# lhaippp/DMHomo

Measured on AMD Instinct MI355X. Metric: sampled images/sec (128x128, s_step=32), higher is better.
Workload: dtype f32; 1 GPU; DGM CFG-Unet dim=64 128x128 bs=25/GPU s_step=32 cond_scale=3 (BASELINE configs[1]); global_batch=25, cfg_mode=streams, hip_graph=True, weights=seeded random init

## Files before the change

dmhomo_amd/csrc/linattn_fused.hip:

```cpp

#include "common.h"

typedef _Float16 half8 __attribute__((ext_vector_type(8)));
typedef _Float16 half4 __attribute__((ext_vector_type(4)));
typedef float float4v __attribute__((ext_vector_type(4)));

#define LA_PART (32 + 32 + 1024)

#ifdef DMH_STAMPS
__device__ int g_la_ablate = 0;
extern "C" int dmh_la_set_ablate(int v) {
  return hipMemcpyToSymbol(HIP_SYMBOL(g_la_ablate), &v, sizeof(int)) == hipSuccess ? 0 : -1;
}
#define LA_ABL_LOAD() const int la_abl = g_la_ablate
#define LA_ABL(bit) ((la_abl >> (bit)) & 1)
#else
#define LA_ABL_LOAD() constexpr int la_abl = 0
#define LA_ABL(bit) 0
#endif

namespace {
constexpr int KC = 32;

__device__ __forceinline__ void la_split2(float x0, float x1, float s, unsigned& h, unsigned& r, int cheap) {
  if (cheap) {
    float t0 = x0 * s, t1 = x1 * s;
    asm("v_cvt_pk_f16_f32 %0, %1, %2" : "=v"(h) : "v"(t0), "v"(t1));
    r = 0u;
  } else {
    dmh_split2(x0, x1, s, h, r);
  }
}
__device__ __forceinline__ void la_split8(const float (&x)[8], float s, dmh_half8& h, dmh_half8& r, int cheap) {
  if (cheap) {
    uint4 hh, rr = make_uint4(0u, 0u, 0u, 0u);
    la_split2(x[0], x[1], s, hh.x, rr.x, 1);
    la_split2(x[2], x[3], s, hh.y, rr.y, 1);
    la_split2(x[4], x[5], s, hh.z, rr.z, 1);
    la_split2(x[6], x[7], s, hh.w, rr.w, 1);
    asm volatile("s_nop 3" : "+v"(hh.x), "+v"(hh.y), "+v"(hh.z), "+v"(hh.w));
    h = __builtin_bit_cast(dmh_half8, hh);
    r = __builtin_bit_cast(dmh_half8, rr);
  } else {
    dmh_split8(x, s, h, r);
  }
}
constexpr int PITCH = 160;
constexpr int TP = 64;
constexpr int TILE_BYTES = TP * PITCH;

__device__ __forceinline__ unsigned absbits(float x) { return __float_as_uint(x) & 0x7fffffffu; }

template <int NBUF>
struct Stager {
  const float* xb;
  const float* g;
  int C, n, p0;
  int c4, pix0;
  float mean[2], rstd[2];
  bool ok[2];
  float4 v[2];
  float4 gq;
  float sc, inv_sc;
  int seq = 0;
  int abl = 0;

  __device__ __forceinline__ void init_scale() {
    float m = 0.f;
    for (int i = threadIdx.x & 63; i < C; i += 64) m = fmaxf(m, fabsf(g[i]));
#pragma unroll
    for (int off = 32; off; off >>= 1) m = fmaxf(m, __shfl_xor(m, off));
    const float bound = m * sqrtf((float)C);
    const int e = min(max((int)(__builtin_amdgcn_readfirstlane(__float_as_uint(bound)) >> 23) & 0xff, 16), 254);
    sc = __uint_as_float((unsigned)(268 - e) << 23);
    inv_sc = __uint_as_float((unsigned)(e - 14) << 23);
  }
  __device__ __forceinline__ void begin_tile(const float* stats_b, int p0_) {
    p0 = p0_;
#pragma unroll
    for (int i = 0; i < 2; ++i) {
      const int pix = p0 + pix0 + 32 * i;
      ok[i] = pix < n;
      const int pc = (abl & 8) ? pix0 : (ok[i] ? pix : n - 1);
      mean[i] = stats_b[(size_t)pc * 2 + 0];
      rstd[i] = stats_b[(size_t)pc * 2 + 1];
    }
  }
  __device__ __forceinline__ void issue(int ch) {
#pragma unroll
    for (int i = 0; i < 2; ++i) {
      const int pix = p0 + pix0 + 32 * i;
      const int pc = (abl & 8) ? pix0 : (pix < n ? pix : n - 1);
      v[i] = ld4(xb + (size_t)pc * C + ch * KC + c4 * 4);
    }
    gq = ld4(g + ch * KC + c4 * 4);
  }
  __device__ __forceinline__ unsigned char* stage(unsigned char* tiles) {
    unsigned char* tile = tiles + (NBUF == 2 ? (seq & 1) * TILE_BYTES : 0);
    ++seq;
    if (NBUF == 1) __syncthreads();
#pragma unroll
    for (int i = 0; i < 2; ++i) {
      float4 x = v[i];
      if (ok[i]) {
        x.x = (x.x - mean[i]) * rstd[i] * gq.x;
        x.y = (x.y - mean[i]) * rstd[i] * gq.y;
        x.z = (x.z - mean[i]) * rstd[i] * gq.z;
        x.w = (x.w - mean[i]) * rstd[i] * gq.w;
      } else {
        x = make_float4(0.f, 0.f, 0.f, 0.f);
      }
      uint2 h1, h2;
      la_split2(x.x, x.y, sc, h1.x, h2.x, abl & 1);
      la_split2(x.z, x.w, sc, h1.y, h2.y, abl & 1);
      unsigned char* dst = tile + (pix0 + 32 * i) * PITCH + c4 * 8;
      *reinterpret_cast<uint2*>(dst) = h1;
      *reinterpret_cast<uint2*>(dst + 64) = h2;
    }
    __syncthreads();
    return tile;
  }
  __device__ __forceinline__ float inv_scale() const { return inv_sc; }
};

__device__ __forceinline__ void dmh_raw_barrier() {
  asm volatile("" ::: "memory");
  __builtin_amdgcn_s_barrier();
  asm volatile("" ::: "memory");
}

struct RingStager {
  static constexpr int RD = 2;
  static constexpr int UNIT = TP * 64 * 4;
  static constexpr int STATS_SLOTS = 4;
  static constexpr int BYTES = RD * UNIT + STATS_SLOTS * TP * 8;
  const float* xb;
  const float* stats_b;
  int n, p0w, U;
  int c4, pix0, lane, wave;
  unsigned char* ring;
  unsigned ring_lds;
  float4 gq[2];
  float sc, inv_sc;
  int seq = 0;
  int abl = 0;

  __device__ __forceinline__ void init(const float* x_b, const float* stats_b_, const float* g, int n_, int p0w_, int tiles,
                                       unsigned char* ring_) {
    xb = x_b;
    stats_b = stats_b_;
    n = n_;
    p0w = p0w_;
    const int left = (n - p0w + TP - 1) / TP;
    U = left < tiles ? left : tiles;
    lane = threadIdx.x & 63;
    wave = __builtin_amdgcn_readfirstlane(threadIdx.x >> 6);
    c4 = threadIdx.x & 7;
    pix0 = threadIdx.x >> 3;
    ring = ring_;
    ring_lds = (unsigned)(size_t)ring_;
    float m = fabsf(g[lane]);
#pragma unroll
    for (int off = 32; off; off >>= 1) m = fmaxf(m, __shfl_xor(m, off));
    const float bound = m * 8.0f;
    const int e = min(max((int)(__builtin_amdgcn_readfirstlane(__float_as_uint(bound)) >> 23) & 0xff, 16), 254);
    sc = __uint_as_float((unsigned)(268 - e) << 23);
    inv_sc = __uint_as_float((unsigned)(e - 14) << 23);
    gq[0] = ld4(g + c4 * 4);
    gq[1] = ld4(g + KC + c4 * 4);
  }
  __device__ __forceinline__ void glds(const void* src, unsigned lds_dst, bool x4) {
    unsigned keep;
    if (x4)
      asm volatile("s_mov_b32 %0, m0\n\ts_mov_b32 m0, %2\n\ts_nop 0\n\tglobal_load_lds_dwordx4 %1, off\n\ts_mov_b32 m0, %0"
                   : "=&s"(keep) : "v"(src), "s"(lds_dst) : "memory");
    else
      asm volatile("s_mov_b32 %0, m0\n\ts_mov_b32 m0, %2\n\ts_nop 0\n\tglobal_load_lds_dword %1, off\n\ts_mov_b32 m0, %0"
                   : "=&s"(keep) : "v"(src), "s"(lds_dst) : "memory");
  }
  __device__ __forceinline__ void issue_unit(int t) {
    const int p0 = (abl & 8) ? 0 : p0w + t * TP;
    const int fl = min((p0 + wave * 16) * 2 + (lane & 31), 2 * n - 1);
    if (lane < 32) glds(stats_b + fl, ring_lds + RD * UNIT + (t % STATS_SLOTS) * (TP * 8) + wave * 128, false);
#pragma unroll
    for (int j = 0; j < 4; ++j) {
      const int piece = wave * 4 + j;
      const int pc = min(p0 + piece * 4 + (lane >> 4), n - 1);
      glds(xb + (size_t)pc * 64 + (lane & 15) * 4, ring_lds + (t % RD) * UNIT + piece * 1024, true);
    }
  }
  __device__ __forceinline__ void prime() {
    if (U > 0) issue_unit(0);
    if (U > 1) {
      issue_unit(1);
      asm volatile("s_waitcnt vmcnt(5)" ::: "memory");
    } else {
      asm volatile("s_waitcnt vmcnt(0)" ::: "memory");
    }
    dmh_raw_barrier();
  }
  __device__ __forceinline__ unsigned char* stage(unsigned char* tiles) {
    const int t = seq++;
    unsigned char* set = tiles + (t & 1) * (2 * TILE_BYTES);
    const unsigned char* raw = ring + (t % RD) * UNIT;
    const int p0 = p0w + t * TP;
    const float* st = reinterpret_cast<const float*>(ring + RD * UNIT + (t % STATS_SLOTS) * (TP * 8));
#pragma unroll
    for (int i = 0; i < 2; ++i) {
      const float2 mr = *reinterpret_cast<const float2*>(st + (pix0 + 32 * i) * 2);
      const bool ok = p0 + pix0 + 32 * i < n;
#pragma unroll
      for (int ch = 0; ch < 2; ++ch) {
        float4 x = *reinterpret_cast<const float4*>(raw + (pix0 + 32 * i) * 256 + ch * 128 + c4 * 16);
        const float4 gv = gq[ch];
        if (ok) {
          x.x = (x.x - mr.x) * mr.y * gv.x;
          x.y = (x.y - mr.x) * mr.y * gv.y;
          x.z = (x.z - mr.x) * mr.y * gv.z;
          x.w = (x.w - mr.x) * mr.y * gv.w;
        } else {
          x = make_float4(0.f, 0.f, 0.f, 0.f);
        }
        uint2 h1, h2;
        la_split2(x.x, x.y, sc, h1.x, h2.x, abl & 1);
        la_split2(x.z, x.w, sc, h1.y, h2.y, abl & 1);
        unsigned char* dst = set + ch * TILE_BYTES + (pix0 + 32 * i) * PITCH + c4 * 8;
        *reinterpret_cast<uint2*>(dst) = h1;
        *reinterpret_cast<uint2*>(dst + 64) = h2;
      }
    }
    return set;
  }
  __device__ __forceinline__ void sync() {
    const int t = seq - 1;
    asm volatile("s_waitcnt lgkmcnt(0)" ::: "memory");
    asm volatile("s_waitcnt vmcnt(0)" ::: "memory");
    dmh_raw_barrier();
    if (t + RD < U) issue_unit(t + RD);
  }
  __device__ __forceinline__ float inv_scale() const { return inv_sc; }
};

}

__global__ __launch_bounds__(256, 2) void linattn_kv_kernel(const float* __restrict__ x, const float* __restrict__ stats,
                                                            const float* __restrict__ g, const uint4* __restrict__ wkv,
                                                            const float* __restrict__ oscale, float* __restrict__ partial,
                                                            int n, int C, int nsplit, int tiles,
                                                            const int32_t* __restrict__ rows) {
  extern __shared__ __attribute__((aligned(16))) unsigned char smem[];
  unsigned char* tiles_lds = smem;

  const int jb = blockIdx.x / nsplit, sp = blockIdx.x % nsplit;
  if (rows && jb >= rows[0]) return;
  const int b = dmh_rows_phys(rows, jb);
  const int tid = threadIdx.x, lane = tid & 63, h = tid >> 6;
  const int l15 = lane & 15, kg = lane >> 4;
  const int nch = C / KC;

  LA_ABL_LOAD();
  Stager<2> st;
  st.abl = la_abl;
  st.xb = x + (size_t)b * n * C;
  st.g = g;
  st.C = C;
  st.n = n;
  st.c4 = tid & 7;
  st.pix0 = tid >> 3;
  st.init_scale();
  const float* stats_b = stats + (size_t)b * n * 2;

  const uint4* wb = wkv + (size_t)h * nch * (8 * 64) + lane;
  float osc[4];
#pragma unroll
  for (int nb = 0; nb < 4; ++nb) osc[nb] = oscale[(h * 4 + nb) * 16 + l15];

  float m_run[2] = {-INFINITY, -INFINITY}, s_run[2] = {0.f, 0.f};
  float4v ctx[2][2];
#pragma unroll
  for (int i = 0; i < 2; ++i)
#pragma unroll
    for (int j = 0; j < 2; ++j) ctx[i][j] = float4v{0.f, 0.f, 0.f, 0.f};

  if (sp * tiles * TP < n) {
    st.begin_tile(stats_b, sp * tiles * TP);
    st.issue(0);
  }
  for (int tI = 0; tI < tiles; ++tI) {
    const int p0 = (sp * tiles + tI) * TP;
    if (p0 >= n) break;
    float4v acc[4][4];
#pragma unroll
    for (int mb = 0; mb < 4; ++mb)
#pragma unroll
      for (int nb = 0; nb < 4; ++nb) acc[mb][nb] = float4v{0.f, 0.f, 0.f, 0.f};

    auto chunk = [&](int ch, const uint4 (&bq)[8]) __attribute__((always_inline)) {
      const unsigned char* tile = st.stage(tiles_lds);
      if (ch + 1 < nch) st.issue(ch + 1);
      half8 a[4][2];
#pragma unroll
      for (int mb = 0; mb < 4; ++mb)
#pragma unroll
        for (int pl = 0; pl < 2; ++pl)
          a[mb][pl] = *reinterpret_cast<const half8*>(tile + (mb * 16 + l15) * PITCH + kg * 16 + pl * 64);
#define LA_TERM(pl, bexpr)                                                                          \
  _Pragma("unroll") for (int mb = 0; mb < 4; ++mb) _Pragma("unroll") for (int nb = 0; nb < 4; ++nb) \
      acc[mb][nb] = __builtin_amdgcn_mfma_f32_16x16x32_f16(a[mb][pl], bexpr, acc[mb][nb], 0, 0, 0);
      if (!LA_ABL(4)) {
      LA_TERM(1, __builtin_bit_cast(half8, bq[nb * 2]))
      LA_TERM(0, __builtin_bit_cast(half8, bq[nb * 2 + 1]))
      LA_TERM(0, __builtin_bit_cast(half8, bq[nb * 2]))
      } else {
        acc[0][0][0] += (float)a[0][0][0] + (float)a[3][1][7];
      }
#undef LA_TERM
    };
    for (int ch = 0; ch < nch; ++ch) {
      uint4 bq[8];
#pragma unroll
      for (int i = 0; i < 8; ++i) bq[i] = wb[(size_t)(ch * 8 + i) * 64];
      chunk(ch, bq);
    }
    const float inv_s = st.inv_scale();
    if (tI + 1 < tiles && p0 + TP < n) {
      st.begin_tile(stats_b, p0 + TP);
      st.issue(0);
    }

    const bool full = p0 + TP <= n;
    float m_new[2];
#pragma unroll
    for (int db = 0; db < 2; ++db) {
      const float kk = inv_s * osc[db] * 1.44269504088896341f;
      float m = -INFINITY;
      if (full) {
#pragma unroll
        for (int mb = 0; mb < 4; ++mb)
#pragma unroll
          for (int r = 0; r < 4; ++r) {
            const float kv = acc[mb][db][r] * kk;
            acc[mb][db][r] = kv;
            m = fmaxf(m, kv);
          }
      } else {
#pragma unroll
        for (int mb = 0; mb < 4; ++mb)
#pragma unroll
          for (int r = 0; r < 4; ++r) {
            const bool valid = p0 + mb * 16 + 4 * kg + r < n;
            const float kv = valid ? acc[mb][db][r] * kk : -INFINITY;
            acc[mb][db][r] = kv;
            m = fmaxf(m, kv);
          }
      }
      m = rows_max(m);
      m_new[db] = fmaxf(m_run[db], m);
    }
#pragma unroll
    for (int db = 0; db < 2; ++db) {
      const float fcol = __builtin_amdgcn_exp2f(m_run[db] - m_new[db]);
      s_run[db] *= fcol;
      ctx[0][db] *= fcol;
      ctx[1][db] *= fcol;
      m_run[db] = m_new[db];
    }
    half8 p1[2][2], p2[2][2], v1[2][2], v2[2][2];
#pragma unroll
    for (int db = 0; db < 2; ++db) {
      float s = 0.f;
#pragma unroll
      for (int ks = 0; ks < 2; ++ks) {
        float pv[8];
#pragma unroll
        for (int j = 0; j < 8; ++j) {
          const float arg = acc[2 * ks + (j >> 2)][db][j & 3] - m_new[db];
          pv[j] = LA_ABL(1) ? arg : __builtin_amdgcn_exp2f(arg);
          s += pv[j];
        }
        la_split8(pv, 1024.f, p1[db][ks], p2[db][ks], LA_ABL(0));
      }
      s = rows_sum(s);
      s_run[db] += s;
    }
    unsigned mx = 0u;
#pragma unroll
    for (int eb = 0; eb < 2; ++eb) {
      const float kv2 = inv_s * osc[2 + eb];
#pragma unroll
      for (int mb = 0; mb < 4; ++mb)
#pragma unroll
        for (int r = 0; r < 4; ++r) {
          const float vv = acc[mb][2 + eb][r] * kv2;
          acc[mb][2 + eb][r] = vv;
          mx = max(mx, absbits(vv));
        }
    }
    mx = wave_max_u32(mx);
    const int exv = min(max((int)(mx >> 23), 32), 254);
    const float scv = __uint_as_float((unsigned)(268 - exv) << 23);
    const float inv_v = __uint_as_float((unsigned)(exv - 14 - 10) << 23);
#pragma unroll
    for (int eb = 0; eb < 2; ++eb)
#pragma unroll
      for (int ks = 0; ks < 2; ++ks) {
        float vv[8];
#pragma unroll
        for (int j = 0; j < 8; ++j) vv[j] = acc[2 * ks + (j >> 2)][2 + eb][j & 3];
        la_split8(vv, scv, v1[eb][ks], v2[eb][ks], LA_ABL(0));
      }
    float4v t[2][2];
#pragma unroll
    for (int eb = 0; eb < 2; ++eb)
#pragma unroll
      for (int db = 0; db < 2; ++db)
        t[eb][db] = __builtin_amdgcn_mfma_f32_16x16x32_f16(v2[eb][0], p1[db][0], float4v{0.f, 0.f, 0.f, 0.f}, 0, 0, 0);
#pragma unroll
    for (int eb = 0; eb < 2; ++eb)
#pragma unroll
      for (int db = 0; db < 2; ++db) t[eb][db] = __builtin_amdgcn_mfma_f32_16x16x32_f16(v2[eb][1], p1[db][1], t[eb][db], 0, 0, 0);
#pragma unroll
    for (int st2 = 0; st2 < 2; ++st2)
#pragma unroll
      for (int eb = 0; eb < 2; ++eb)
#pragma unroll
        for (int db = 0; db < 2; ++db)
          t[eb][db] = __builtin_amdgcn_mfma_f32_16x16x32_f16(v1[eb][st2], p2[db][st2], t[eb][db], 0, 0, 0);
#pragma unroll
    for (int st2 = 0; st2 < 2; ++st2)
#pragma unroll
      for (int eb = 0; eb < 2; ++eb)
#pragma unroll
        for (int db = 0; db < 2; ++db)
          t[eb][db] = __builtin_amdgcn_mfma_f32_16x16x32_f16(v1[eb][st2], p1[db][st2], t[eb][db], 0, 0, 0);
#pragma unroll
    for (int eb = 0; eb < 2; ++eb)
#pragma unroll
      for (int db = 0; db < 2; ++db) ctx[eb][db] += t[eb][db] * inv_v;
  }

  float* out = partial + ((size_t)(b * nsplit + sp) * 4 + h) * LA_PART;
  if (kg == 0) {
#pragma unroll
    for (int db = 0; db < 2; ++db) {
      out[db * 16 + l15] = m_run[db] * 0.693147180559945309f;
      out[32 + db * 16 + l15] = s_run[db];
    }
  }
#pragma unroll
  for (int db = 0; db < 2; ++db)
#pragma unroll
    for (int eb = 0; eb < 2; ++eb)
      st4(out + 64 + (db * 16 + l15) * 32 + eb * 16 + 4 * kg,
          make_float4(ctx[eb][db][0], ctx[eb][db][1], ctx[eb][db][2], ctx[eb][db][3]));
}

__global__ __launch_bounds__(256, 2) void linattn_kv_ring_kernel(const float* __restrict__ x, const float* __restrict__ stats,
                                                            const float* __restrict__ g, const uint4* __restrict__ wkv,
                                                            const float* __restrict__ oscale, float* __restrict__ partial,
                                                            int n, int C, int nsplit, int tiles,
                                                            const int32_t* __restrict__ rows) {
  extern __shared__ __attribute__((aligned(16))) unsigned char smem[];
  unsigned char* tiles_lds = smem;
  constexpr int RES = 2;

  const int jb = blockIdx.x / nsplit, sp = blockIdx.x % nsplit;
  if (rows && jb >= rows[0]) return;
  const int b = dmh_rows_phys(rows, jb);
  const int tid = threadIdx.x, lane = tid & 63, h = tid >> 6;
  const int l15 = lane & 15, kg = lane >> 4;

  LA_ABL_LOAD();
  RingStager st;
  st.abl = la_abl;
  st.init(x + (size_t)b * n * C, stats + (size_t)b * n * 2, g, n, sp * tiles * TP, tiles, smem + 4 * TILE_BYTES);
  const int nch = 2;

  const uint4* wb = wkv + (size_t)h * nch * (8 * 64) + lane;
  float osc[4];
#pragma unroll
  for (int nb = 0; nb < 4; ++nb) osc[nb] = oscale[(h * 4 + nb) * 16 + l15];

  float m_run[2] = {-INFINITY, -INFINITY}, s_run[2] = {0.f, 0.f};
  float4v ctx[2][2];
#pragma unroll
  for (int i = 0; i < 2; ++i)
#pragma unroll
    for (int j = 0; j < 2; ++j) ctx[i][j] = float4v{0.f, 0.f, 0.f, 0.f};

  uint4 wres[RES ? RES : 1][8];
  if (RES) {
#pragma unroll
    for (int ch = 0; ch < RES; ++ch)
#pragma unroll
      for (int i = 0; i < 8; ++i) wres[ch][i] = wb[(size_t)(ch * 8 + i) * 64];
  }
#pragma unroll
  for (int ch = 0; ch < RES; ++ch)
#pragma unroll
    for (int i = 0; i < 8; ++i) asm volatile("" ::"v"(wres[ch][i].x), "v"(wres[ch][i].y), "v"(wres[ch][i].z), "v"(wres[ch][i].w));
  asm volatile("" ::"v"(st.gq[0].x), "v"(st.gq[0].y), "v"(st.gq[0].z), "v"(st.gq[0].w), "v"(st.gq[1].x), "v"(st.gq[1].y),
               "v"(st.gq[1].z), "v"(st.gq[1].w), "v"(osc[0]), "v"(osc[1]), "v"(osc[2]), "v"(osc[3]));
  st.prime();
#ifdef DMH_STAMPS
  unsigned long long tk[6] = {0, 0, 0, 0, 0, 0}, t_prev, t_now;
#define KSTAMP(i)                                                                \
// ... 188 lines not shown
                                                            const float* __restrict__ oscale, const float* __restrict__ ctxm,
                                                            float* __restrict__ out, int n, int C, int nblk, int tiles,
                                                            float scale, FuseOut fo, const int32_t* __restrict__ rows) {
  extern __shared__ __attribute__((aligned(16))) unsigned char smem[];
  constexpr int NBUF = FUSE ? 1 : 2;
  unsigned char* tiles_lds = smem;
  float* yx = reinterpret_cast<float*>(smem + TILE_BYTES);

  const int jb = blockIdx.x / nblk, blk = blockIdx.x % nblk;
  if (rows && jb >= rows[0]) return;
  const int b = dmh_rows_phys(rows, jb);
  const int tid = threadIdx.x, lane = tid & 63, h = tid >> 6;
  const int l15 = lane & 15, kg = lane >> 4;
  const int nch = C / KC;

  LA_ABL_LOAD();
  Stager<NBUF> st;
  st.abl = la_abl;
  st.xb = x + (size_t)b * n * C;
  st.g = g;
  st.C = C;
  st.n = n;
  st.c4 = tid & 7;
  st.pix0 = tid >> 3;
  st.init_scale();
  const float* stats_b = stats + (size_t)b * n * 2;

  const uint4* wb = wq + (size_t)h * nch * (4 * 64) + lane;
  float osc[2][4];
  half8 c1[2], c2[2];
  float inv_c, mo = 1.f, inv_o = 1.f;
  {
    const float* cb = ctxm + (size_t)(b * 4 + h) * 1024;
    float cv[2][8];
    unsigned mx = 0u;
#pragma unroll
    for (int db = 0; db < 2; ++db)
#pragma unroll
      for (int r = 0; r < 4; ++r) {
        const int d = db * 16 + 4 * kg + r;
        osc[db][r] = oscale[h * 32 + d];
#pragma unroll
        for (int eb = 0; eb < 2; ++eb) {
          cv[eb][db * 4 + r] = cb[d * 32 + eb * 16 + l15];
          mx = max(mx, absbits(cv[eb][db * 4 + r]));
        }
      }
    mx = wave_max_u32(mx);
    const int ex = min(max((int)(mx >> 23), 32), 254);
    const float scc = __uint_as_float((unsigned)(268 - ex) << 23);
    inv_c = __uint_as_float((unsigned)(ex - 14 - 17) << 23);
#pragma unroll
    for (int eb = 0; eb < 2; ++eb) dmh_split8(cv[eb], scc, c1[eb], c2[eb]);
    if (FUSE) {
      unsigned* xm = reinterpret_cast<unsigned*>(yx);
      if (lane == 0) xm[h] = mx;
      __syncthreads();
      const unsigned ma = max(max(xm[0], xm[1]), max(xm[2], xm[3]));
      const float bo = __uint_as_float(ma) * scale;
      const int exo = min(max((int)(__float_as_uint(bo) >> 23) + 1, 16), 254);
      mo = inv_c * __uint_as_float((unsigned)(268 - exo) << 23);
      inv_o = __uint_as_float((unsigned)(exo - 14) << 23);
    }
  }
  float* ob = out + (size_t)b * n * 128 + h * 32;
  half8 wo1[4], wo2[4];
  if (FUSE) {
#pragma unroll
    for (int cb = 0; cb < 4; ++cb) {
      wo1[cb] = __builtin_bit_cast(half8, fo.wo[((h * 4 + cb) * 2 + 0) * 64 + lane]);
      wo2[cb] = __builtin_bit_cast(half8, fo.wo[((h * 4 + cb) * 2 + 1) * 64 + lane]);
    }
  }

  if (blk * tiles * TP < n) {
    st.begin_tile(stats_b, blk * tiles * TP);
    st.issue(0);
  }
  uint4 wres[2][4];
  if (FUSE) {
#pragma unroll
    for (int ch = 0; ch < 2; ++ch)
#pragma unroll
      for (int i = 0; i < 4; ++i) wres[ch][i] = wb[(size_t)(ch * 4 + i) * 64];
  }
#ifdef DMH_STAMPS
  unsigned long long tk[6] = {0, 0, 0, 0, 0, 0}, t_prev, t_now;
#define LSTAMP(i)                                                                \
  __builtin_amdgcn_sched_barrier(0);                                             \
  asm volatile("s_memtime %0\n\ts_waitcnt lgkmcnt(0)" : "=s"(t_now)::"memory"); \
  __builtin_amdgcn_sched_barrier(0);                                             \
  tk[i] += t_now - t_prev;                                                       \
  t_prev = t_now;
  asm volatile("s_memtime %0\n\ts_waitcnt lgkmcnt(0)" : "=s"(t_prev)::"memory");
#else
#define LSTAMP(i)
#endif
  for (int tI = 0; tI < tiles; ++tI) {
    const int p0 = (blk * tiles + tI) * TP;
    if (p0 >= n) break;
    float4v acc[2][4];
#pragma unroll
    for (int db = 0; db < 2; ++db)
#pragma unroll
      for (int nbn = 0; nbn < 4; ++nbn) acc[db][nbn] = float4v{0.f, 0.f, 0.f, 0.f};

    auto chunk = [&](int ch, const uint4 (&aq)[4]) __attribute__((always_inline)) {
      const unsigned char* tile = st.stage(tiles_lds);
      if (ch + 1 < nch) st.issue(ch + 1);
      half8 xb[4][2];
#pragma unroll
      for (int nbn = 0; nbn < 4; ++nbn)
#pragma unroll
        for (int pl = 0; pl < 2; ++pl)
          xb[nbn][pl] = *reinterpret_cast<const half8*>(tile + (nbn * 16 + l15) * PITCH + kg * 16 + pl * 64);
#define LA_TERM(aexpr, pl)                                                                           \
  _Pragma("unroll") for (int db = 0; db < 2; ++db) _Pragma("unroll") for (int nbn = 0; nbn < 4; ++nbn) \
      acc[db][nbn] = __builtin_amdgcn_mfma_f32_16x16x32_f16(aexpr, xb[nbn][pl], acc[db][nbn], 0, 0, 0);
      if (!LA_ABL(4)) {
      LA_TERM(__builtin_bit_cast(half8, aq[db * 2]), 1)
      LA_TERM(__builtin_bit_cast(half8, aq[db * 2 + 1]), 0)
      LA_TERM(__builtin_bit_cast(half8, aq[db * 2]), 0)
      } else {
        acc[0][0][0] += (float)xb[0][0][0] + (float)xb[3][1][7];
      }
#undef LA_TERM
    };
    if (FUSE) {
#pragma unroll
      for (int ch = 0; ch < 2; ++ch) chunk(ch, wres[ch]);
    } else {
      for (int ch = 0; ch < nch; ++ch) {
        uint4 aq[4];
#pragma unroll
        for (int i = 0; i < 4; ++i) aq[i] = wb[(size_t)(ch * 4 + i) * 64];
        chunk(ch, aq);
      }
    }
    const float inv_s = st.inv_scale();
    float qsc[2][4];
#pragma unroll
    for (int db = 0; db < 2; ++db)
#pragma unroll
      for (int r = 0; r < 4; ++r) qsc[db][r] = inv_s * osc[db][r] * 1.44269504088896341f;
    if (tI + 1 < tiles && p0 + TP < n) {
      st.begin_tile(stats_b, p0 + TP);
      st.issue(0);
    }

    LSTAMP(0)
    float rsv[4];
#pragma unroll
    for (int nbn = 0; nbn < 4; ++nbn) {
      float m = -INFINITY;
#pragma unroll
      for (int db = 0; db < 2; ++db)
#pragma unroll
        for (int r = 0; r < 4; ++r) {
          const float qv = acc[db][nbn][r] * qsc[db][r];
          acc[db][nbn][r] = qv;
          m = fmaxf(m, qv);
        }
      m = rows_max(m);
      float s = 0.f;
#pragma unroll
      for (int db = 0; db < 2; ++db)
#pragma unroll
        for (int r = 0; r < 4; ++r) {
          const float e = LA_ABL(1) ? acc[db][nbn][r] - m : __builtin_amdgcn_exp2f(acc[db][nbn][r] - m);
          acc[db][nbn][r] = e;
          s += e;
        }
      s = rows_sum(s);
      rsv[nbn] = scale * 131072.f * __builtin_amdgcn_rcpf(s);
    }
    LSTAMP(1)
    float4v yacc[4][4];
    half8 q1[4], q2[4];
#pragma unroll
    for (int nbn = 0; nbn < 4; ++nbn) {
      float e8[8];
#pragma unroll
      for (int j = 0; j < 8; ++j) e8[j] = acc[j >> 2][nbn][j & 3];
      la_split8(e8, rsv[nbn], q1[nbn], q2[nbn], LA_ABL(0));
    }
    float4v ot[4][2];
#pragma unroll
    for (int nbn = 0; nbn < 4; ++nbn)
#pragma unroll
      for (int eb = 0; eb < 2; ++eb)
        ot[nbn][eb] = __builtin_amdgcn_mfma_f32_16x16x32_f16(c1[eb], q2[nbn], float4v{0.f, 0.f, 0.f, 0.f}, 0, 0, 0);
#pragma unroll
    for (int nbn = 0; nbn < 4; ++nbn)
#pragma unroll
      for (int eb = 0; eb < 2; ++eb)
        ot[nbn][eb] = __builtin_amdgcn_mfma_f32_16x16x32_f16(c2[eb], q1[nbn], ot[nbn][eb], 0, 0, 0);
#pragma unroll
    for (int nbn = 0; nbn < 4; ++nbn)
#pragma unroll
      for (int eb = 0; eb < 2; ++eb)
        ot[nbn][eb] = __builtin_amdgcn_mfma_f32_16x16x32_f16(c1[eb], q1[nbn], ot[nbn][eb], 0, 0, 0);
    if (FUSE) {
      asm volatile("s_nop 7"
                   : "+v"(ot[0][0]), "+v"(ot[0][1]), "+v"(ot[1][0]), "+v"(ot[1][1]), "+v"(ot[2][0]), "+v"(ot[2][1]),
                     "+v"(ot[3][0]), "+v"(ot[3][1]));
      half8 h1[4], h2[4];
#pragma unroll
      for (int nbn = 0; nbn < 4; ++nbn) {
        float o8[8];
#pragma unroll
        for (int j = 0; j < 8; ++j) o8[j] = ot[nbn][j >> 2][j & 3];
        la_split8(o8, mo, h1[nbn], h2[nbn], LA_ABL(0));
      }
#pragma unroll
      for (int nbn = 0; nbn < 4; ++nbn)
#pragma unroll
        for (int cb = 0; cb < 4; ++cb) yacc[cb][nbn] = __builtin_amdgcn_mfma_f32_16x16x32_f16(wo1[cb], h2[nbn], float4v{0.f, 0.f, 0.f, 0.f}, 0, 0, 0);
#pragma unroll
      for (int nbn = 0; nbn < 4; ++nbn)
#pragma unroll
        for (int cb = 0; cb < 4; ++cb) yacc[cb][nbn] = __builtin_amdgcn_mfma_f32_16x16x32_f16(wo2[cb], h1[nbn], yacc[cb][nbn], 0, 0, 0);
#pragma unroll
      for (int nbn = 0; nbn < 4; ++nbn)
#pragma unroll
        for (int cb = 0; cb < 4; ++cb) yacc[cb][nbn] = __builtin_amdgcn_mfma_f32_16x16x32_f16(wo1[cb], h1[nbn], yacc[cb][nbn], 0, 0, 0);
    } else {
#pragma unroll
      for (int nbn = 0; nbn < 4; ++nbn) {
        const int pix = p0 + nbn * 16 + l15;
        if (pix < n) {
#pragma unroll
          for (int eb = 0; eb < 2; ++eb) {
            const float4v o = ot[nbn][eb] * inv_c;
            st4(ob + (size_t)pix * 128 + eb * 16 + 4 * kg, make_float4(o[0], o[1], o[2], o[3]));
          }
        }
      }
    }
    LSTAMP(2)
    if (FUSE) {
#pragma unroll
      for (int cb = 0; cb < 4; ++cb)
#pragma unroll
        for (int nbn = 0; nbn < 4; ++nbn)
          st4(yx + ((h * TP) + nbn * 16 + l15) * YP + cb * 16 + 4 * kg,
              make_float4(yacc[cb][nbn][0], yacc[cb][nbn][1], yacc[cb][nbn][2], yacc[cb][nbn][3]));
      const int quad = tid & 15;
      float4 xr[4];
#pragma unroll
      for (int i = 0; i < 4; ++i) {
        const int pix = LA_ABL(3) ? (tid >> 4) : min(p0 + (tid >> 4) + 16 * i, n - 1);
        xr[i] = ld4(st.xb + (size_t)pix * 64 + quad * 4);
      }
      float4 oq = ld4(fo.osc_o + quad * 4);
      const float4 bq4 = ld4(fo.bias + quad * 4), gq4 = ld4(fo.g_out + quad * 4);
      oq.x *= inv_o;
      oq.y *= inv_o;
      oq.z *= inv_o;
      oq.w *= inv_o;
      __syncthreads();
      LSTAMP(3)
#pragma unroll
      for (int i = 0; i < 4; ++i) {
        if (LA_ABL(2)) break;
        const int pl = (tid >> 4) + 16 * i;
        const float* yp = yx + pl * YP + quad * 4;
        const float4 y0 = ld4(yp), y1 = ld4(yp + TP * YP), y2 = ld4(yp + 2 * TP * YP), y3 = ld4(yp + 3 * TP * YP);
        float4 v;
        v.x = fmaf((y0.x + y1.x) + (y2.x + y3.x), oq.x, bq4.x);
        v.y = fmaf((y0.y + y1.y) + (y2.y + y3.y), oq.y, bq4.y);
        v.z = fmaf((y0.z + y1.z) + (y2.z + y3.z), oq.z, bq4.z);
        v.w = fmaf((y0.w + y1.w) + (y2.w + y3.w), oq.w, bq4.w);
        float sm = (v.x + v.y) + (v.z + v.w);
        sm = row16_sum(sm);
        const float mean = sm / 64.f;
        const float dx = v.x - mean, dy = v.y - mean, dz = v.z - mean, dw = v.w - mean;
        float qs = (dx * dx + dy * dy) + (dz * dz + dw * dw);
        qs = row16_sum(qs);
        const float rs = __builtin_amdgcn_rsqf(qs * (1.f / 64.f) + fo.eps);
        const int pix = p0 + pl;
        if (pix < n) {
          float4 r4;
          r4.x = dx * rs * gq4.x + xr[i].x;
          r4.y = dy * rs * gq4.y + xr[i].y;
          r4.z = dz * rs * gq4.z + xr[i].z;
          r4.w = dw * rs * gq4.w + xr[i].w;
          st4(fo.y + ((size_t)b * n + pix) * 64 + quad * 4, r4);
        }
      }
    }
    LSTAMP(4)
    if (FUSE) __syncthreads();
    LSTAMP(5)
  }
#ifdef DMH_STAMPS
  if (FUSE && lane == 0) {
    float* d = fo.y + ((size_t)b * n + (size_t)blk * tiles * TP) * 64 + h * 8;
    for (int i = 0; i < 6; ++i) d[i] = (float)tk[i];
  }
#endif
}
#undef LSTAMP

__global__ __launch_bounds__(64) void linattn_wscale_kernel(const float* __restrict__ w, float* __restrict__ osc_q,
                                                            float* __restrict__ osc_kv, int C) {
  const int row = blockIdx.x;
  float m = 0.f;
  for (int i = threadIdx.x; i < C; i += 64) m = fmaxf(m, fabsf(w[(size_t)row * C + i]));
  for (int off = 32; off; off >>= 1) m = fmaxf(m, __shfl_xor(m, off));
  if (threadIdx.x == 0) {
    float s = 1.f;
    if (m > 0.f && m < 3.0e38f) {
      int e;
      frexpf(m, &e);
      s = ldexpf(1.f, min(max(e - 15, -100), 100));
    }
    if (row < 128) {
      osc_q[row] = s;
    } else {
      const int part = row / 128 - 1, hh = (row % 128) / 32, d = row % 32;
      osc_kv[(hh * 4 + part * 2 + d / 16) * 16 + d % 16] = s;
    }
  }
}

__global__ void linattn_pack_kernel(const float* __restrict__ w, const float* __restrict__ osc_q,
                                    const float* __restrict__ osc_kv, _Float16* __restrict__ pq,
                                    _Float16* __restrict__ pkv, int C, int64_t total_q, int64_t total_kv) {
  const int64_t idx = (int64_t)blockIdx.x * blockDim.x + threadIdx.x;
  const int nch = C / KC;
  if (idx < total_q) {
    int64_t r = idx;
    const int j = r % 8;
    r /= 8;
    const int lane = r % 64;
    r /= 64;
    const int plane = r % 2;
    r /= 2;
    const int db = r % 2;
    r /= 2;
    const int ch = r % nch;
    const int hh = r / nch;
    const int row = hh * 32 + db * 16 + (lane & 15);
    const int c = ch * KC + (lane >> 4) * 8 + j;
    const float ws = w[(size_t)row * C + c] / osc_q[row];
    const _Float16 g1 = (_Float16)ws;
    pq[idx] = plane == 0 ? g1 : (_Float16)(ws - (float)g1);
  }
  if (idx < total_kv) {
    int64_t r = idx;
    const int j = r % 8;
    r /= 8;
    const int lane = r % 64;
    r /= 64;
    const int plane = r % 2;
    r /= 2;
    const int nb = r % 4;
    r /= 4;
    const int ch = r % nch;
    const int hh = r / nch;
    const int row = 128 + (nb >> 1) * 128 + hh * 32 + (nb & 1) * 16 + (lane & 15);
    const int c = ch * KC + (lane >> 4) * 8 + j;
    const float ws = w[(size_t)row * C + c] / osc_kv[(hh * 4 + nb) * 16 + (lane & 15)];
    const _Float16 g1 = (_Float16)ws;
    pkv[idx] = plane == 0 ? g1 : (_Float16)(ws - (float)g1);
  }
}

extern "C" int64_t dmh_linattn_fused_pack_floats(int C) { if (!dmh_dims_ok({C})) return -1; return (int64_t)C * 128 + (int64_t)C * 256 + 128 + 256; }

extern "C" int dmh_linattn_fused_pack(const float* w_qkv, float* wpack, int C, void* stream) {
  DMH_REQUIRE(w_qkv && wpack && C > 0 && C % KC == 0, "dmh_linattn_fused_pack: C must be a multiple of 32 (got %d)", C);
  hipStream_t s = (hipStream_t)stream;
  float* osc_q = wpack + (int64_t)C * 384;
  float* osc_kv = osc_q + 128;
  hipLaunchKernelGGL(linattn_wscale_kernel, dim3(384), dim3(64), 0, s, w_qkv, osc_q, osc_kv, C);
  const int64_t total_q = (int64_t)C * 128 * 2, total_kv = (int64_t)C * 256 * 2;
  hipLaunchKernelGGL(linattn_pack_kernel, dim3((unsigned)cdiv64(total_kv, 256)), dim3(256), 0, s, w_qkv, osc_q, osc_kv,
                     reinterpret_cast<_Float16*>(wpack), reinterpret_cast<_Float16*>(wpack + (int64_t)C * 128), C,
                     total_q, total_kv);
  DMH_CHECK_LAUNCH("dmh_linattn_fused_pack");
  return DMH_OK;
}

static int fused_tiles(int B, int n) {
  (void)B;
  const int nt = cdiv(n, TP);
  const int t = nt / 32;
  return t < 1 ? 1 : (t > 8 ? 8 : t);
}

extern "C" int dmh_linattn_fused_splits(int B, int n) {
  if (!dmh_dims_ok({B}) || !dmh_dims_ok({n}, 1, 1 << 26)) return -1;
  return cdiv(cdiv(n, TP), fused_tiles(B, n));
}

extern "C" int dmh_linattn_fused_context(const float* x, const float* stats, const float* ln_g, const float* wpack,
                                         float* partial, int B, int n, int C, const int32_t* rows, void* stream) {
  DMH_REQUIRE(x && stats && ln_g && wpack && partial, "dmh_linattn_fused_context: null pointer");
  DMH_REQUIRE(B > 0 && n > 0 && C > 0 && C % KC == 0, "dmh_linattn_fused_context: bad shape (C=%d)", C);
  const int tiles = fused_tiles(B, n), nsplit = cdiv(cdiv(n, TP), tiles);
  const uint4* wkv = reinterpret_cast<const uint4*>(wpack + (int64_t)C * 128);
  const float* osc_kv = wpack + (int64_t)C * 384 + 128;
  if (C == 2 * KC) {
    constexpr int LDS = 4 * TILE_BYTES + RingStager::BYTES;
    DMH_RAISE_LDS_ONCE(linattn_kv_ring_kernel, LDS, "dmh_linattn_fused_context");
    hipLaunchKernelGGL(linattn_kv_ring_kernel, dim3(B * nsplit), dim3(256), LDS, (hipStream_t)stream, x, stats, ln_g, wkv,
                       osc_kv, partial, n, C, nsplit, tiles, rows);
  } else
    hipLaunchKernelGGL(linattn_kv_kernel, dim3(B * nsplit), dim3(256), 2 * TILE_BYTES, (hipStream_t)stream, x, stats, ln_g,
                       wkv, osc_kv, partial, n, C, nsplit, tiles, rows);
  DMH_CHECK_LAUNCH("dmh_linattn_fused_context");
  return DMH_OK;
}

extern "C" int dmh_linattn_fused_apply(const float* x, const float* stats, const float* ln_g, const float* wpack,
                                       const float* ctx, float* out, int B, int n, int C, float scale, const int32_t* rows,
                                       void* stream) {
  DMH_REQUIRE(x && stats && ln_g && wpack && ctx && out, "dmh_linattn_fused_apply: null pointer");
  DMH_REQUIRE(B > 0 && n > 0 && C > 0 && C % KC == 0, "dmh_linattn_fused_apply: bad shape (C=%d)", C);
  const int tiles = fused_tiles(B, n), nblk = cdiv(cdiv(n, TP), tiles);
  const uint4* wq = reinterpret_cast<const uint4*>(wpack);
  const float* osc_q = wpack + (int64_t)C * 384;
  FuseOut fo = {};
  hipLaunchKernelGGL(linattn_qo_kernel<false>, dim3(B * nblk), dim3(256), 2 * TILE_BYTES, (hipStream_t)stream, x, stats,
                     ln_g, wq, osc_q, ctx, out, n, C, nblk, tiles, scale, fo, rows);
  DMH_CHECK_LAUNCH("dmh_linattn_fused_apply");
  return DMH_OK;
}

__global__ __launch_bounds__(64) void linattn_wo_scale_kernel(const float* __restrict__ w, float* __restrict__ osc) {
  const int c = blockIdx.x;
  float m = fmaxf(fabsf(w[c * 128 + threadIdx.x]), fabsf(w[c * 128 + 64 + threadIdx.x]));
  for (int off = 32; off; off >>= 1) m = fmaxf(m, __shfl_xor(m, off));
  if (threadIdx.x == 0) {
    float s = 1.f;
    if (m > 0.f && m < 3.0e38f) {
      int e;
      frexpf(m, &e);
      s = ldexpf(1.f, min(max(e - 15, -100), 100));
    }
    osc[c] = s;
  }
}
__global__ void linattn_wo_pack_kernel(const float* __restrict__ w, const float* __restrict__ osc,
                                       _Float16* __restrict__ wp) {
  const int idx = blockIdx.x * blockDim.x + threadIdx.x;
  if (idx >= 16384) return;
  int r = idx;
  const int j = r % 8;
  r /= 8;
  const int lane = r % 64;
  r /= 64;
  const int plane = r % 2;
  r /= 2;
  const int cb = r % 4;
  const int hh = r / 4;
  const int c = cb * 16 + (lane & 15), kg = lane >> 4;
  const int e = j < 4 ? 4 * kg + j : 16 + 4 * kg + (j - 4);
  const float ws = w[c * 128 + hh * 32 + e] / osc[c];
  const _Float16 g1 = (_Float16)ws;
  wp[idx] = plane == 0 ? g1 : (_Float16)(ws - (float)g1);
}

extern "C" int64_t dmh_linattn_out_pack_floats(void) { return 16384 / 2 + 64; }

extern "C" int dmh_linattn_out_pack(const float* w_out, float* wpack, void* stream) {
  DMH_REQUIRE(w_out && wpack, "dmh_linattn_out_pack: null pointer");
  hipStream_t s = (hipStream_t)stream;
  hipLaunchKernelGGL(linattn_wo_scale_kernel, dim3(64), dim3(64), 0, s, w_out, wpack + 8192);
  hipLaunchKernelGGL(linattn_wo_pack_kernel, dim3(64), dim3(256), 0, s, w_out, wpack + 8192,
                     reinterpret_cast<_Float16*>(wpack));
  DMH_CHECK_LAUNCH("dmh_linattn_out_pack");
  return DMH_OK;
}

extern "C" int dmh_linattn_fused_apply_out(const float* x, const float* stats, const float* ln_g, const float* wpack,
                                           const float* ctx, const float* wopack, const float* out_bias,
                                           const float* out_ln_g, float* y, int B, int n, int C, float scale,
                                           float eps, const int32_t* rows, void* stream) {
  DMH_REQUIRE(x && stats && ln_g && wpack && ctx && wopack && out_bias && out_ln_g && y,
              "dmh_linattn_fused_apply_out: null pointer");
  DMH_REQUIRE(B > 0 && n > 0 && C == 64, "dmh_linattn_fused_apply_out: only C == 64 (got %d)", C);
  const int tiles = fused_tiles(B, n), nblk = cdiv(cdiv(n, TP), tiles);
  const uint4* wq = reinterpret_cast<const uint4*>(wpack);
  const float* osc_q = wpack + (int64_t)C * 384;
  FuseOut fo;
  fo.wo = reinterpret_cast<const uint4*>(wopack);
  fo.osc_o = wopack + 8192;
  fo.bias = out_bias;
  fo.g_out = out_ln_g;
  fo.y = y;
  fo.eps = eps;
  constexpr int LDS = TILE_BYTES + YX_BYTES;
  DMH_RAISE_LDS_ONCE(linattn_qo_kernel<true>, LDS, "dmh_linattn_fused_apply_out");
  hipLaunchKernelGGL(linattn_qo_kernel<true>, dim3(B * nblk), dim3(256), LDS, (hipStream_t)stream, x, stats, ln_g, wq,
                     osc_q, ctx, nullptr, n, C, nblk, tiles, scale, fo, rows);
  DMH_CHECK_LAUNCH("dmh_linattn_fused_apply_out");
  return DMH_OK;
}
```

Before: 89.71 images/s.

## Add ring-staged fused linear-attention output kernel with single tile set and aliased LDS

Adds a new fused Q/softmax/context/output-projection/LayerNorm kernel that stages input through the ring stager with a single tile set. The output exchange buffer is aliased over the staged tiles and processed in two halves, cutting LDS so two workgroups fit per CU, and the next unit's loads are issued right after the QK MFMAs. The fused apply_out entry point now launches this kernel instead of the old qo kernel. The trade-off is less double-buffering overlap and extra barriers per tile in return for higher occupancy.

Result: no change. 90.22 images/s, median of 6 (+0.6%).

```diff
diff --git a/dmhomo_amd/csrc/linattn_fused.hip b/dmhomo_amd/csrc/linattn_fused.hip
--- a/dmhomo_amd/csrc/linattn_fused.hip
+++ b/dmhomo_amd/csrc/linattn_fused.hip
@@ -199,9 +199,10 @@
     }
     dmh_raw_barrier();
   }
+  template <int SETS = 2>
   __device__ __forceinline__ unsigned char* stage(unsigned char* tiles) {
     const int t = seq++;
-    unsigned char* set = tiles + (t & 1) * (2 * TILE_BYTES);
+    unsigned char* set = tiles + (SETS == 2 ? (t & 1) * (2 * TILE_BYTES) : 0);
     const unsigned char* raw = ring + (t % RD) * UNIT;
     const int p0 = p0w + t * TP;
     const float* st = reinterpret_cast<const float*>(ring + RD * UNIT + (t % STATS_SLOTS) * (TP * 8));
@@ -996,6 +997,289 @@
 }
 #undef LSTAMP
 
+constexpr int YR = TP / 2;
+constexpr int YR_BYTES = 4 * YR * YP * 4;
+constexpr int QO_RING_LDS = YR_BYTES + RingStager::BYTES;
+static_assert(2 * TILE_BYTES + 16 <= YR_BYTES, "the staged set (and the head maxima behind it) lie under the exchange buffer");
+static_assert(2 * QO_RING_LDS <= 160 * 1024, "two workgroups per CU");
+
+__global__ __launch_bounds__(256, 2) void linattn_qo_ring_kernel(const float* __restrict__ x, const float* __restrict__ stats,
+                                                                 const float* __restrict__ g, const uint4* __restrict__ wq,
+                                                                 const float* __restrict__ oscale,
+                                                                 const float* __restrict__ ctxm, int n, int nblk, int tiles,
+                                                                 float scale, FuseOut fo, const int32_t* __restrict__ rows) {
+  extern __shared__ __attribute__((aligned(16))) unsigned char smem[];
+  unsigned char* tiles_lds = smem;
+  float* yx = reinterpret_cast<float*>(smem);
+
+  const int jb = blockIdx.x / nblk, blk = blockIdx.x % nblk;
+  if (rows && jb >= rows[0]) return;
+  const int b = dmh_rows_phys(rows, jb);
+  const int tid = threadIdx.x, lane = tid & 63, h = tid >> 6;
+  const int l15 = lane & 15, kg = lane >> 4;
+  const int quad = tid & 15, prow = tid >> 4;
+
+  LA_ABL_LOAD();
+  RingStager st;
+  st.abl = la_abl;
+  st.init(x + (size_t)b * n * 64, stats + (size_t)b * n * 2, g, n, blk * tiles * TP, tiles, smem + YR_BYTES);
+
+  const uint4* wb = wq + (size_t)h * 2 * (4 * 64) + lane;
+  float osc[2][4];
+  half8 c1[2], c2[2];
+  float inv_c, mo, inv_o;
+  unsigned mx = 0u;
+  {
+    const float* cb = ctxm + (size_t)(b * 4 + h) * 1024;
+    float cv[2][8];
+#pragma unroll
+    for (int db = 0; db < 2; ++db)
+#pragma unroll
+      for (int r = 0; r < 4; ++r) {
+        const int d = db * 16 + 4 * kg + r;
+        osc[db][r] = oscale[h * 32 + d];
+#pragma unroll
+        for (int eb = 0; eb < 2; ++eb) {
+          cv[eb][db * 4 + r] = cb[d * 32 + eb * 16 + l15];
+          mx = max(mx, absbits(cv[eb][db * 4 + r]));
+        }
+      }
+    mx = wave_max_u32(mx);
+    const int ex = min(max((int)(mx >> 23), 32), 254);
+    const float scc = __uint_as_float((unsigned)(268 - ex) << 23);
+    inv_c = __uint_as_float((unsigned)(ex - 14 - 17) << 23);
+#pragma unroll
+    for (int eb = 0; eb < 2; ++eb) dmh_split8(cv[eb], scc, c1[eb], c2[eb]);
+  }
+  half8 wo1[4], wo2[4];
+#pragma unroll
+  for (int cb = 0; cb < 4; ++cb) {
+    wo1[cb] = __builtin_bit_cast(half8, fo.wo[((h * 4 + cb) * 2 + 0) * 64 + lane]);
+    wo2[cb] = __builtin_bit_cast(half8, fo.wo[((h * 4 + cb) * 2 + 1) * 64 + lane]);
+  }
+  uint4 wres[2][4];
+#pragma unroll
+  for (int ch = 0; ch < 2; ++ch)
+#pragma unroll
+    for (int i = 0; i < 4; ++i) wres[ch][i] = wb[(size_t)(ch * 4 + i) * 64];
+  float4 oq = ld4(fo.osc_o + quad * 4);
+  const float4 bq4 = ld4(fo.bias + quad * 4), gq4 = ld4(fo.g_out + quad * 4);
+#pragma unroll
+  for (int ch = 0; ch < 2; ++ch)
+#pragma unroll
+    for (int i = 0; i < 4; ++i) asm volatile("" ::"v"(wres[ch][i].x), "v"(wres[ch][i].y), "v"(wres[ch][i].z), "v"(wres[ch][i].w));
+#pragma unroll
+  for (int cb = 0; cb < 4; ++cb) asm volatile("" ::"v"(wo1[cb]), "v"(wo2[cb]));
+  asm volatile("" ::"v"(st.gq[0].x), "v"(st.gq[0].y), "v"(st.gq[0].z), "v"(st.gq[0].w), "v"(st.gq[1].x), "v"(st.gq[1].y),
+               "v"(st.gq[1].z), "v"(st.gq[1].w), "v"(c1[0]), "v"(c1[1]), "v"(c2[0]), "v"(c2[1]));
+  asm volatile("" ::"v"(oq.x), "v"(oq.y), "v"(oq.z), "v"(oq.w), "v"(bq4.x), "v"(bq4.y), "v"(bq4.z), "v"(bq4.w), "v"(gq4.x),
+               "v"(gq4.y), "v"(gq4.z), "v"(gq4.w), "v"(osc[0][0]), "v"(osc[0][1]), "v"(osc[0][2]), "v"(osc[0][3]),
+               "v"(osc[1][0]), "v"(osc[1][1]), "v"(osc[1][2]), "v"(osc[1][3]));
+  unsigned* xm = reinterpret_cast<unsigned*>(smem + 2 * TILE_BYTES);
+  if (lane == 0) xm[h] = mx;
+  asm volatile("s_waitcnt vmcnt(0) lgkmcnt(0)" ::: "memory");
+  if (st.U > 0) st.issue_unit(0);
+  asm volatile("s_waitcnt vmcnt(0)" ::: "memory");
+  dmh_raw_barrier();
+  {
+    const unsigned ma = max(max(xm[0], xm[1]), max(xm[2], xm[3]));
+    const float bo = __uint_as_float(ma) * scale;
+    const int exo = min(max((int)(__float_as_uint(bo) >> 23) + 1, 16), 254);
+    mo = inv_c * __uint_as_float((unsigned)(268 - exo) << 23);
+    inv_o = __uint_as_float((unsigned)(exo - 14) << 23);
+  }
+  oq.x *= inv_o;
+  oq.y *= inv_o;
+  oq.z *= inv_o;
+  oq.w *= inv_o;
+  const float inv_s = st.inv_scale();
+  float qsc[2][4];
+#pragma unroll
+  for (int db = 0; db < 2; ++db)
+#pragma unroll
+    for (int r = 0; r < 4; ++r) qsc[db][r] = inv_s * osc[db][r] * 1.44269504088896341f;
+
+#ifdef DMH_STAMPS
+  unsigned long long tk[6] = {0, 0, 0, 0, 0, 0}, t_prev, t_now;
+#define LSTAMP(i)                                                                \
+  __builtin_amdgcn_sched_barrier(0);                                             \
+  asm volatile("s_memtime %0\n\ts_waitcnt lgkmcnt(0)" : "=s"(t_now)::"memory"); \
+  __builtin_amdgcn_sched_barrier(0);                                             \
+  tk[i] += t_now - t_prev;                                                       \
+  t_prev = t_now;
+  asm volatile("s_memtime %0\n\ts_waitcnt lgkmcnt(0)" : "=s"(t_prev)::"memory");
+#else
+#define LSTAMP(i)
+#endif
+  for (int tI = 0; tI < st.U; ++tI) {
+    const int p0 = st.p0w + tI * TP;
+    const unsigned char* raw = st.ring + (tI % RingStager::RD) * RingStager::UNIT;
+    float4v acc[2][4];
+#pragma unroll
+    for (int db = 0; db < 2; ++db)
+#pragma unroll
+      for (int nbn = 0; nbn < 4; ++nbn) acc[db][nbn] = float4v{0.f, 0.f, 0.f, 0.f};
+
+    const unsigned char* set = st.stage<1>(tiles_lds);
+    asm volatile("s_waitcnt lgkmcnt(0)" ::: "memory");
+    dmh_raw_barrier();
+#pragma unroll
+    for (int ch = 0; ch < 2; ++ch) {
+      const unsigned char* tile = set + ch * TILE_BYTES;
+      half8 xb[4][2];
+#pragma unroll
+      for (int nbn = 0; nbn < 4; ++nbn)
+#pragma unroll
+        for (int pl = 0; pl < 2; ++pl)
+          xb[nbn][pl] = *reinterpret_cast<const half8*>(tile + (nbn * 16 + l15) * PITCH + kg * 16 + pl * 64);
+#define LA_TERM(aexpr, pl)                                                                           \
+  _Pragma("unroll") for (int db = 0; db < 2; ++db) _Pragma("unroll") for (int nbn = 0; nbn < 4; ++nbn) \
+      acc[db][nbn] = __builtin_amdgcn_mfma_f32_16x16x32_f16(aexpr, xb[nbn][pl], acc[db][nbn], 0, 0, 0);
+      if (!LA_ABL(4)) {
+      LA_TERM(__builtin_bit_cast(half8, wres[ch][db * 2]), 1)
+      LA_TERM(__builtin_bit_cast(half8, wres[ch][db * 2 + 1]), 0)
+      LA_TERM(__builtin_bit_cast(half8, wres[ch][db * 2]), 0)
+      } else {
+        acc[0][0][0] += (float)xb[0][0][0] + (float)xb[3][1][7];
+      }
+#undef LA_TERM
+    }
+    asm volatile("s_waitcnt lgkmcnt(0)" ::: "memory");
+    dmh_raw_barrier();
+    if (tI + 1 < st.U) st.issue_unit(tI + 1);
+
+    LSTAMP(0)
+    float rsv[4];
+#pragma unroll
+    for (int nbn = 0; nbn < 4; ++nbn) {
+      float m = -INFINITY;
+#pragma unroll
+      for (int db = 0; db < 2; ++db)
+#pragma unroll
+        for (int r = 0; r < 4; ++r) {
+          const float qv = acc[db][nbn][r] * qsc[db][r];
+          acc[db][nbn][r] = qv;
+          m = fmaxf(m, qv);
+        }
+      m = rows_max(m);
+      float s = 0.f;
+#pragma unroll
+      for (int db = 0; db < 2; ++db)
+#pragma unroll
+        for (int r = 0; r < 4; ++r) {
+          const float e = LA_ABL(1) ? acc[db][nbn][r] - m : __builtin_amdgcn_exp2f(acc[db][nbn][r] - m);
+          acc[db][nbn][r] = e;
+          s += e;
+        }
+      s = rows_sum(s);
+      rsv[nbn] = scale * 131072.f * __builtin_amdgcn_rcpf(s);
+    }
+    LSTAMP(1)
+    float4v yacc[4][4];
+    half8 q1[4], q2[4];
+#pragma unroll
+    for (int nbn = 0; nbn < 4; ++nbn) {
+      float e8[8];
+#pragma unroll
+      for (int j = 0; j < 8; ++j) e8[j] = acc[j >> 2][nbn][j & 3];
+      la_split8(e8, rsv[nbn], q1[nbn], q2[nbn], LA_ABL(0));
+    }
+    float4v ot[4][2];
+#pragma unroll
+    for (int nbn = 0; nbn < 4; ++nbn)
+#pragma unroll
+      for (int eb = 0; eb < 2; ++eb)
+        ot[nbn][eb] = __builtin_amdgcn_mfma_f32_16x16x32_f16(c1[eb], q2[nbn], float4v{0.f, 0.f, 0.f, 0.f}, 0, 0, 0);
+#pragma unroll
+    for (int nbn = 0; nbn < 4; ++nbn)
+#pragma unroll
+      for (int eb = 0; eb < 2; ++eb)
+        ot[nbn][eb] = __builtin_amdgcn_mfma_f32_16x16x32_f16(c2[eb], q1[nbn], ot[nbn][eb], 0, 0, 0);
+#pragma unroll
+    for (int nbn = 0; nbn < 4; ++nbn)
+#pragma unroll
+      for (int eb = 0; eb < 2; ++eb)
+        ot[nbn][eb] = __builtin_amdgcn_mfma_f32_16x16x32_f16(c1[eb], q1[nbn], ot[nbn][eb], 0, 0, 0);
+    asm volatile("s_nop 7"
+                 : "+v"(ot[0][0]), "+v"(ot[0][1]), "+v"(ot[1][0]), "+v"(ot[1][1]), "+v"(ot[2][0]), "+v"(ot[2][1]),
+                   "+v"(ot[3][0]), "+v"(ot[3][1]));
+    half8 h1[4], h2[4];
+#pragma unroll
+    for (int nbn = 0; nbn < 4; ++nbn) {
+      float o8[8];
+#pragma unroll
+      for (int j = 0; j < 8; ++j) o8[j] = ot[nbn][j >> 2][j & 3];
+      la_split8(o8, mo, h1[nbn], h2[nbn], LA_ABL(0));
+    }
+#pragma unroll
+    for (int nbn = 0; nbn < 4; ++nbn)
+#pragma unroll
+      for (int cb = 0; cb < 4; ++cb) yacc[cb][nbn] = __builtin_amdgcn_mfma_f32_16x16x32_f16(wo1[cb], h2[nbn], float4v{0.f, 0.f, 0.f, 0.f}, 0, 0, 0);
+#pragma unroll
+    for (int nbn = 0; nbn < 4; ++nbn)
+#pragma unroll
+      for (int cb = 0; cb < 4; ++cb) yacc[cb][nbn] = __builtin_amdgcn_mfma_f32_16x16x32_f16(wo2[cb], h1[nbn], yacc[cb][nbn], 0, 0, 0);
+#pragma unroll
+    for (int nbn = 0; nbn < 4; ++nbn)
+#pragma unroll
+      for (int cb = 0; cb < 4; ++cb) yacc[cb][nbn] = __builtin_amdgcn_mfma_f32_16x16x32_f16(wo1[cb], h1[nbn], yacc[cb][nbn], 0, 0, 0);
+    LSTAMP(2)
+#pragma unroll
+    for (int rd = 0; rd < 2; ++rd) {
+#pragma unroll
+      for (int cb = 0; cb < 4; ++cb)
+#pragma unroll
+        for (int k = 0; k < 2; ++k)
+          st4(yx + ((h * YR) + k * 16 + l15) * YP + cb * 16 + 4 * kg,
+              make_float4(yacc[cb][2 * rd + k][0], yacc[cb][2 * rd + k][1], yacc[cb][2 * rd + k][2], yacc[cb][2 * rd + k][3]));
+      asm volatile("s_waitcnt vmcnt(0) lgkmcnt(0)" ::: "memory");
+      dmh_raw_barrier();
+      if (rd == 0) { LSTAMP(3) }
+#pragma unroll
+      for (int k = 0; k < 2; ++k) {
+        if (LA_ABL(2)) break;
+        const int pr = prow + 16 * k;
+        const int pl = YR * rd + pr;
+        const float* yp = yx + pr * YP + quad * 4;
+        const float4 y0 = ld4(yp), y1 = ld4(yp + YR * YP), y2 = ld4(yp + 2 * YR * YP), y3 = ld4(yp + 3 * YR * YP);
+        const float4 xr = *reinterpret_cast<const float4*>(raw + pl * 256 + quad * 16);
+        float4 v;
+        v.x = fmaf((y0.x + y1.x) + (y2.x + y3.x), oq.x, bq4.x);
+        v.y = fmaf((y0.y + y1.y) + (y2.y + y3.y), oq.y, bq4.y);
+        v.z = fmaf((y0.z + y1.z) + (y2.z + y3.z), oq.z, bq4.z);
+        v.w = fmaf((y0.w + y1.w) + (y2.w + y3.w), oq.w, bq4.w);
+        float sm = (v.x + v.y) + (v.z + v.w);
+        sm = row16_sum(sm);
+        const float mean = sm / 64.f;
+        const float dx = v.x - mean, dy = v.y - mean, dz = v.z - mean, dw = v.w - mean;
+        float qs = (dx * dx + dy * dy) + (dz * dz + dw * dw);
+        qs = row16_sum(qs);
+        const float rs = __builtin_amdgcn_rsqf(qs * (1.f / 64.f) + fo.eps);
+        const int pix = p0 + pl;
+        if (pix < n) {
+          float4 r4;
+          r4.x = dx * rs * gq4.x + xr.x;
+          r4.y = dy * rs * gq4.y + xr.y;
+          r4.z = dz * rs * gq4.z + xr.z;
+          r4.w = dw * rs * gq4.w + xr.w;
+          st4(fo.y + ((size_t)b * n + pix) * 64 + quad * 4, r4);
+        }
+      }
+      if (rd == 1) { LSTAMP(4) }
+      asm volatile("s_waitcnt vmcnt(0) lgkmcnt(0)" ::: "memory");
+      dmh_raw_barrier();
+    }
+    LSTAMP(5)
+  }
+#ifdef DMH_STAMPS
+  if (lane == 0) {
+    float* d = fo.y + ((size_t)b * n + (size_t)blk * tiles * TP) * 64 + h * 8;
+    for (int i = 0; i < 6; ++i) d[i] = (float)tk[i];
+  }
+#endif
+}
+#undef LSTAMP
+
 __global__ __launch_bounds__(64) void linattn_wscale_kernel(const float* __restrict__ w, float* __restrict__ osc_q,
                                                             float* __restrict__ osc_kv, int C) {
   const int row = blockIdx.x;
@@ -1186,10 +1470,9 @@
   fo.g_out = out_ln_g;
   fo.y = y;
   fo.eps = eps;
-  constexpr int LDS = TILE_BYTES + YX_BYTES;
-  DMH_RAISE_LDS_ONCE(linattn_qo_kernel<true>, LDS, "dmh_linattn_fused_apply_out");
-  hipLaunchKernelGGL(linattn_qo_kernel<true>, dim3(B * nblk), dim3(256), LDS, (hipStream_t)stream, x, stats, ln_g, wq,
-                     osc_q, ctx, nullptr, n, C, nblk, tiles, scale, fo, rows);
+  DMH_RAISE_LDS_ONCE(linattn_qo_ring_kernel, QO_RING_LDS, "dmh_linattn_fused_apply_out");
+  hipLaunchKernelGGL(linattn_qo_ring_kernel, dim3(B * nblk), dim3(256), QO_RING_LDS, (hipStream_t)stream, x, stats, ln_g, wq,
+                     osc_q, ctx, n, nblk, tiles, scale, fo, rows);
   DMH_CHECK_LAUNCH("dmh_linattn_fused_apply_out");
   return DMH_OK;
 }
```
